# neoncloud/mdctGAN

Hardware: AMD Instinct MI355X
Metric: train steps/sec (G+D) VCTK 12k->48k (higher is better)
Workload: dtype f32; 1 GPU; configs[1]: netG=global ngf=64 n_blocks_global=9 n_blocks_attn_g=0 num_D=2, per-GPU batch 8 x 32512 samples (128 frames x 256 bins), 12k->48k, fp32; global_batch=8, segment_length=32512, parallelism=dp1, launch=hipGraph replay

## Files before the change

include/mdctgan_hip.h:

```cpp
#ifndef MDCTGAN_HIP_H
#define MDCTGAN_HIP_H

#include <stddef.h>

#ifdef __cplusplus
extern "C" {
#endif

#define MG_OK 0
#define MG_ERR_ARG (-1)
#define MG_ERR_UNSUPPORTED (-2)

#define MG_CODEC_RAW 0
#define MG_CODEC_ARCSINH 1
#define MG_CODEC_RANGE 2

#define MG_ACT_NONE 0
#define MG_ACT_RELU 1
#define MG_ACT_LRELU02 2
#define MG_ACT_TANH 3

int mg_abi_version(void);
int mg_conv_geom_size(void);

// ... 195 lines not shown
int mg_conv_fwd_instnorm_w(const mg_conv_geom* g, const float* x, const float* w, const float* bias, float* y_raw, float eps,
                           int act, const float* residual, float* y, float* mean, float* rstd, void* workspace,
                           size_t workspace_bytes, void* stream, const mg_wino_tiles* wt);
int mg_conv_wino_md_from_norm_ok(const mg_conv_geom* g);
int mg_instnorm_bwd_wino_md(const mg_conv_geom* g, const float* gy, const float* y_raw, const float* mean, const float* rstd,
                            int act, float* md, void* stream);
int mg_conv_fwd_instnorm_h(const mg_conv_geom* g, const float* x, const float* w, const float* bias, float* y_raw, float eps,
                           int act, const float* residual, float* y, float* mean, float* rstd, void* workspace,
                           size_t workspace_bytes, void* stream, const mg_wino_tiles* tiles, void* y16);
int mg_conv_wino_vnext_ok(const mg_conv_geom* g);
int mg_conv_fwd_instnorm_next(const mg_conv_geom* g, const float* x, const float* w, const float* bias, float* y_raw, float eps,
                              int act, const float* residual, float* y, float* mean, float* rstd, void* workspace,
                              size_t workspace_bytes, void* stream, const mg_wino_tiles* tiles, float* v_next, int next_reflect);
int mg_conv_dgrad_w(const mg_conv_geom* g, const float* dy, const float* w, const float* bias, float* dx, int act,
                    void* workspace, size_t workspace_bytes, void* stream, const mg_wino_tiles* tiles);
int mg_conv_wgrad(const mg_conv_geom* g, const float* x, const float* dy, float* dw, float* dbias, int accumulate,
                  void* workspace, size_t workspace_bytes, void* stream);
size_t mg_conv_wgrad_workspace(const mg_conv_geom* g);
int mg_conv_wgrad_w(const mg_conv_geom* g, const float* x, const float* dy, float* dw, float* dbias, int accumulate,
                    void* workspace, size_t workspace_bytes, void* stream, const mg_wino_tiles* tiles);
int mg_conv_wgrad_checks_finite(const mg_conv_geom* g);
int mg_conv_wgrad_chk(const mg_conv_geom* g, const float* x, const float* dy, float* dw, float* dbias, int accumulate,
                      void* workspace, size_t workspace_bytes, void* stream, const mg_wino_tiles* tiles, float* found_inf);
int mg_conv_wgrad_h16_ok(const mg_conv_geom* g);
int mg_conv_wgrad_h16(const mg_conv_geom* g, const float* x, const float* dy, void* dw16, int accumulate, void* workspace,
                      size_t workspace_bytes, void* stream, float* found_inf);
typedef struct {
    float* m;
    float* v;
    float* u;
// ... 128 lines not shown
```

mdctgan_amd/_lib.py:

```python
from __future__ import annotations

import ctypes as C
import os

import torch

_HERE = os.path.dirname(os.path.abspath(__file__))
LIB_PATH = os.environ.get("MDCTGAN_HIP_LIB", os.path.join(_HERE, "libmdctgan_hip.so"))

MG_CODEC_RAW, MG_CODEC_ARCSINH, MG_CODEC_RANGE, MG_CODEC_DB, MG_CODEC_EXPLICIT = 0, 1, 2, 3, 4
ACT_NONE, ACT_RELU, ACT_LRELU02, ACT_TANH = 0, 1, 2, 3


class HipLibraryError(RuntimeError):
    pass


class ConvGeom(C.Structure):
    _fields_ = [(n, C.c_int) for n in
                ("B", "H", "W", "Ci", "OH", "OW", "Co", "KH", "KW", "stride", "pad", "reflect", "precision")]


PRECISION_F32, PRECISION_F16 = 0, 1

# ... 7 lines not shown


_W = C.POINTER(WinoTiles)


class LossItem(C.Structure):
    _fields_ = [("a", C.c_void_p), ("b", C.c_void_p), ("grad", C.c_void_p), ("n", C.c_longlong), ("zero_tail", C.c_longlong)]


class WinoAdam(C.Structure):
    _fields_ = [("m", C.c_void_p), ("v", C.c_void_p), ("u", C.c_void_p), ("state", C.c_void_p),
                ("beta1", C.c_float), ("beta2", C.c_float), ("eps", C.c_float), ("grad_scale", C.c_float)]


_WA = C.POINTER(WinoAdam)


class ResampleBank(C.Structure):
    _fields_ = [("kern", C.c_void_p), ("orig", C.c_int), ("new_", C.c_int), ("width", C.c_int)]


_RB = C.POINTER(ResampleBank)

SIGNATURES = {
    "mg_abi_version": (_i, []),
    "mg_conv_geom_size": (_i, []),
    "mg_mdct4_forward": (_i, [_p, _i, _i, _i, _p, _p, _p, _i, _f, _f, _f, _f, _f, _i, _p, _p, _p, _p, _p, _p, _p, _p]),
    "mg_mdct4_num_frames": (_i, [_i, _i]),
    "mg_dct4_image": (_i, [_p, _p, _p]),
    "mg_dct4_image_floats": (_ll, [_i]),
# ... 13 lines not shown
    "mg_imdct4_pow2_stitched": (_i, [_p, _i, _i, _i, _p, _p, _i, _f, _f, _f, _f, _f, _p, _p, _p, _ll, _i, _i, _ll, _i, _i, _p]),
    "mg_conv_fwd": (_i, [_G, _p, _p, _p, _p, _i, _p, _sz, _p]),
    "mg_conv_fwd_workspace": (_sz, [_G]),
    "mg_conv_wino_weights_bytes": (_sz, [_G]),
    "mg_conv_wino_prepare": (_i, [_G, _p, _p, _p]),
    "mg_conv_wino_tiles_bytes": (_sz, [_G, _i]),
    "mg_conv_fwd_w": (_i, [_G, _p, _p, _p, _p, _i, _p, _sz, _p, _W]),
    "mg_conv_fwd_instnorm_workspace": (_sz, [_G]),
    "mg_conv_wino_md_from_norm_ok": (_i, [_G]),
    "mg_instnorm_bwd_wino_md": (_i, [_G, _p, _p, _p, _p, _i, _p, _p]),
    "mg_conv_fwd_instnorm_w": (_i, [_G, _p, _p, _p, _p, _f, _i, _p, _p, _p, _p, _p, _sz, _p, _W]),
    "mg_conv_fwd_instnorm_h": (_i, [_G, _p, _p, _p, _p, _f, _i, _p, _p, _p, _p, _p, _sz, _p, _W, _p]),
    "mg_conv_fwd_instnorm_next": (_i, [_G, _p, _p, _p, _p, _f, _i, _p, _p, _p, _p, _p, _sz, _p, _W, _p, _i]),
    "mg_conv_wino_vnext_ok": (_i, [_G]),
    "mg_conv_dgrad_w": (_i, [_G, _p, _p, _p, _p, _i, _p, _sz, _p, _W]),
    "mg_conv_wgrad_w": (_i, [_G, _p, _p, _p, _p, _i, _p, _sz, _p, _W]),
    "mg_conv_wgrad_chk": (_i, [_G, _p, _p, _p, _p, _i, _p, _sz, _p, _W, _p]),
    "mg_conv_wgrad_checks_finite": (_i, [_G]),
    "mg_conv_wgrad_adam_ok": (_i, [_G]),
    "mg_conv_wgrad_adam_w": (_i, [_G, _p, _p, _p, _WA, _p, _sz, _p, _W]),
    "mg_conv_dgrad": (_i, [_G, _p, _p, _p, _p, _i, _p, _sz, _p]),
    "mg_conv_dgrad_workspace": (_sz, [_G]),
    "mg_conv_wgrad": (_i, [_G, _p, _p, _p, _p, _i, _p, _sz, _p]),
    "mg_conv_wgrad_workspace": (_sz, [_G]),
    "mg_conv_plan_name": (_i, [_i, _G, C.c_char_p, _i]),
    "mg_conv_plan_splits": (_i, [_i, _G]),
    "mg_conv_plan_order": (_i, [_i, _G, C.POINTER(C.c_int), C.POINTER(C.c_int)]),
    "mg_conv_plan_flops": (C.c_double, [_i, _G]),
    "mg_probe_arm": (None, [_p, _p]),
    "mg_resample_length": (_ll, [_ll, _i, _i]),
# ... 192 lines not shown
```

mdctgan_amd/csrc/conv_igemm.hip:

```cpp
#include "common.h"
#include "mdctgan_hip.h"
#include "internal.h"
#include <stdio.h>
#include <stdlib.h>
#include <cstring>
#include <type_traits>
#include <map>
#include <mutex>
#include <tuple>
#include <hip/hip_ext.h>

namespace {

constexpr int BK = 16;

struct Geom {
    int B, H, W, Ci, OH, OW, Co, KH, KW, s, p, reflect;
};

struct Batch {
    long long sa, sw, so;
    int wino_perm;
};
__device__ __forceinline__ int wino_flip(int z) {
// ... 1573 lines not shown
    }
    const dim3 grid(wino_grid((size_t)w.T * g->Co / w.f.vec));
    if (w.r == R_WINO)
        hipLaunchKernelGGL(wino_output_xform_kernel, grid, dim3(256), 0, st, (const float*)Mx, g->B, w.TH, w.TW, g->Co, bias, act, y,
                           (int)w.hp);
    else if (w.r == R_WINO4)
        hipLaunchKernelGGL(wino4_output_xform_kernel, grid, dim3(256), 0, st, (const float*)Mx, g->B, w.TH, w.TW, g->Co, bias, act, y);
    else
        hipLaunchKernelGGL(wino42_output_xform_kernel, grid, dim3(256), 0, st, (const float*)Mx, g->B, g->OH, g->OW, w.TH, w.TW, g->Co,
                           bias, act, y);
    MG_CHECK_LAUNCH();
    return MG_OK;
}

int wino_dgrad(const WinoGeo& w, const mg_conv_geom* g, const float* dy, const float* wt, const float* bias, float* dx, int act,
               float* ws, hipStream_t st, const float* u_pre, float* md_keep, const float** addend) {
    const WinoGemm s = wino_gemm_plan(w, 1, g);
    const WinoWs o = wino_ws(w, s, 1, g);
    float* U = u_pre ? const_cast<float*>(u_pre) : ws + o.u;
    float* Md = md_keep ? md_keep : ws + o.md;
    float* dV = ws + o.dv;
    float* dd = ws + o.dd;
    if (!u_pre) wino_xform_u(w, g, wt, U, st);
    if (dy) wino_xform_md(w, g, dy, Md, st);
    wino_gemm(w, s, 1, g, Md, U, dV, ws + o.part, st);
    if (w.r == R_WINO && !w.hp && wino_dd_gather_ok(g->H, g->W, g->Ci)) {
        const int ts = w.TH * w.TW;
        const size_t lds = (size_t)ts * 16 * 8 * sizeof(float4);
        const dim3 grid(g->Ci / 32, g->B);
        const float* add = *addend;
        *addend = nullptr;
        auto go = [&](auto kern) {
            hipFuncSetAttribute((const void*)kern, hipFuncAttributeMaxDynamicSharedMemorySize, (int)lds);
            hipLaunchKernelGGL(kern, grid, dim3(256), lds, st, (const float*)dV, g->B, g->H, g->W, g->Ci, g->reflect, bias, act, dx, add);
        };
        if (ts <= 32) go(wino_dd_gather_kernel<1>); else go(wino_dd_gather_kernel<2>);
        MG_CHECK_LAUNCH();
        return MG_OK;
    }
    const dim3 grid(wino_grid((size_t)w.T * w.Kc / w.f.vec)), gx(wino_grid((size_t)g->B * g->H * g->W * g->Ci / 4));
    if (w.r == R_WINO) {
        hipLaunchKernelGGL(wino_dd_xform_kernel, grid, dim3(256), 0, st, (const float*)dV, w.T, w.Kc, dd);
        hipLaunchKernelGGL(wino_dx_gather_kernel, gx, dim3(256), 0, st, (const float*)dd, g->B, g->H, g->W, g->Ci, g->reflect, bias,
                           act, dx, (int)w.hp);
    } else {
        hipLaunchKernelGGL(wino4_dd_xform_kernel, grid, dim3(256), 0, st, (const float*)dV, w.T, w.Kc, dd);
        if (w.r == R_WINO4)
            hipLaunchKernelGGL(wino4_dx_gather_kernel, gx, dim3(256), 0, st, (const float*)dd, g->B, g->H, g->W, g->Ci, w.TH, w.TW, dx);
        else
            hipLaunchKernelGGL(wino42_dx_gather_kernel, gx, dim3(256), 0, st, (const float*)dd, g->B, g->H, g->W, g->Ci, w.TH, w.TW, dx);
    }
    MG_CHECK_LAUNCH();
    return MG_OK;
}
// ... 360 lines not shown
int mg_instnorm_bwd_wino_md(const mg_conv_geom* g, const float* gy, const float* y_raw, const float* mean, const float* rstd,
                            int act, float* md, void* stream) {
    if (!gy || !y_raw || !mean || !rstd || !md) return MG_ERR_ARG;
    if (!mg_conv_wino_md_from_norm_ok(g)) return MG_ERR_UNSUPPORTED;
    if (act != MG_ACT_NONE && act != MG_ACT_RELU && act != MG_ACT_LRELU02) return MG_ERR_UNSUPPORTED;
    if (!aligned16(gy) || !aligned16(y_raw) || !aligned16(mean) || !aligned16(rstd) || !aligned16(md)) return MG_ERR_ARG;
    const WinoGeo d = wino_geo(R_WINO, g);
    const dim3 grid(g->Co / 32, g->B);
    const int nt = (d.TH * d.TW + 31) / 32;
    hipStream_t st = (hipStream_t)stream;
#define MG_NORM_BWD_DY(NT_) hipLaunchKernelGGL(wino_norm_bwd_dy_kernel<NT_>, grid, dim3(256), 0, st, gy, y_raw, mean, rstd, g->B, d.TH, d.TW, g->Co, act, md)
    if (nt == 1) MG_NORM_BWD_DY(1); else if (nt == 2) MG_NORM_BWD_DY(2); else if (nt == 3) MG_NORM_BWD_DY(3); else if (nt == 4) MG_NORM_BWD_DY(4); else MG_NORM_BWD_DY(5);
#undef MG_NORM_BWD_DY
    MG_CHECK_LAUNCH();
    return MG_OK;
}
size_t mg_conv_fwd_instnorm_workspace(const mg_conv_geom* g) {
    if (!geom_ok(g)) return 0;
    const size_t a = mg_conv_fwd_workspace(g), b = mg_instnorm_workspace(g->B, g->OH * g->OW, g->Co);
    return a > b ? a : b;
}
int mg_conv_fwd_instnorm_w(const mg_conv_geom* g, const float* x, const float* w, const float* bias, float* y_raw, float eps,
                           int act, const float* residual, float* y, float* mean, float* rstd, void* workspace,
                           size_t workspace_bytes, void* stream, const mg_wino_tiles* wt) {
    return mg_conv_fwd_instnorm_h(g, x, w, bias, y_raw, eps, act, residual, y, mean, rstd, workspace, workspace_bytes, stream, wt, nullptr);
}
static bool wino_vnext_ok(const mg_conv_geom* g) {
    return wino_norm_ok(g) && wino_out_norm_next_ok(g->OH / 2, g->OW / 2, g->Co) && g->Co % 16 == 0;
}
int mg_conv_wino_vnext_ok(const mg_conv_geom* g) { return g && wino_vnext_ok(g) ? 1 : 0; }
// ... 436 lines not shown
```

mdctgan_amd/csrc/wino.h:

```cpp
#pragma once
#include "adam.h"

namespace {

__device__ __forceinline__ void bt4(const float4 d0, const float4 d1, const float4 d2, const float4 d3, float4 (&o)[4]) {
    o[0] = make_float4(d0.x - d2.x, d0.y - d2.y, d0.z - d2.z, d0.w - d2.w);
    o[1] = make_float4(d1.x + d2.x, d1.y + d2.y, d1.z + d2.z, d1.w + d2.w);
    o[2] = make_float4(d2.x - d1.x, d2.y - d1.y, d2.z - d1.z, d2.w - d1.w);
    o[3] = make_float4(d1.x - d3.x, d1.y - d3.y, d1.z - d3.z, d1.w - d3.w);
}
__device__ __forceinline__ float4 f4add(float4 a, float4 b) { return make_float4(a.x + b.x, a.y + b.y, a.z + b.z, a.w + b.w); }
__device__ __forceinline__ float4 f4sub(float4 a, float4 b) { return make_float4(a.x - b.x, a.y - b.y, a.z - b.z, a.w - b.w); }
__device__ __forceinline__ float4 f4scale(float4 a, float s) { return make_float4(a.x * s, a.y * s, a.z * s, a.w * s); }
__device__ __forceinline__ float4 f4neg(float4 a) { return make_float4(-a.x, -a.y, -a.z, -a.w); }

__global__ void wino_input_xform_kernel(const float* __restrict__ x, int B, int H, int W, int C, int TH, int TW,
                                        int org, int reflect, float* __restrict__ V) {
    const int C4 = C / 4;
    const size_t T = (size_t)B * TH * TW, total = T * C4;
    for (size_t i = (size_t)blockIdx.x * blockDim.x + threadIdx.x; i < total; i += (size_t)gridDim.x * blockDim.x) {
        const int c4 = (int)(i % C4);
        const size_t t = i / C4;
        const int tx = (int)(t % TW), ty = (int)((t / TW) % TH), b = (int)(t / ((size_t)TW * TH));
        float4 d[4][4];
// ... 246 lines not shown
                }
#pragma unroll
                for (int r = 0; r < 4; ++r) {
                    float4 o[4];
                    bt4(tmp[r][0], tmp[r][1], tmp[r][2], tmp[r][3], o);
#pragma unroll
                    for (int c = 0; c < 4; ++c)
                        *reinterpret_cast<float4*>(nrm.v_next + ((size_t)(r * 4 + c) * T + t) * C + c0) = o[c];
                }
            }
        }
    }
}
inline bool wino_out_norm_next_ok(int TH, int TW, int C) { return C % 32 == 0 && TH * TW <= 64; }

template <int NT>
__global__ __launch_bounds__(256) void wino_norm_bwd_dy_kernel(const float* __restrict__ gy, const float* __restrict__ x,
                                                               const float* __restrict__ mean, const float* __restrict__ rstd,
                                                               int B, int TH, int TW, int C, int act, float* __restrict__ Md) {
    __shared__ double red[2][32][32];
    const int cq = threadIdx.x & 7, tl = threadIdx.x >> 3;
    const int b = blockIdx.y, c0 = blockIdx.x * 32 + 4 * cq;
    const int Ts = TH * TW, HW = 4 * Ts;
    const size_t T = (size_t)B * Ts;
    const float4 mu4 = ld4(mean + (size_t)b * C + c0), rs4 = ld4(rstd + (size_t)b * C + c0);
    const float mu[4] = {mu4.x, mu4.y, mu4.z, mu4.w}, rs[4] = {rs4.x, rs4.y, rs4.z, rs4.w};
    float xh[NT][4][4], gq[NT][4][4];
    double s1[4] = {0, 0, 0, 0}, s2[4] = {0, 0, 0, 0};
#pragma unroll
    for (int i = 0; i < NT; ++i) {
        const int tile = tl + 32 * i;
        if (tile < Ts) {
            const int ty = tile / TW, tx = tile - ty * TW;
#pragma unroll
            for (int q = 0; q < 4; ++q) {
                const size_t off = ((size_t)(b * 2 * TH + 2 * ty + (q >> 1)) * (2 * TW) + 2 * tx + (q & 1)) * C + c0;
                float xv[4], gv[4];
                *reinterpret_cast<float4*>(xv) = ld4(x + off);
                *reinterpret_cast<float4*>(gv) = ld4(gy + off);
#pragma unroll
                for (int j = 0; j < 4; ++j) {
                    xh[i][q][j] = (xv[j] - mu[j]) * rs[j];
                    const float d = act == MG_ACT_RELU ? (xh[i][q][j] > 0.0f ? 1.0f : 0.0f)
                                  : act == MG_ACT_LRELU02 ? (xh[i][q][j] > 0.0f ? 1.0f : 0.2f) : 1.0f;
                    gq[i][q][j] = gv[j] * d;
                    s1[j] += (double)gq[i][q][j];
                    s2[j] += (double)gq[i][q][j] * (double)xh[i][q][j];
                }
            }
        } else {
#pragma unroll
            for (int q = 0; q < 4; ++q)
#pragma unroll
                for (int j = 0; j < 4; ++j) xh[i][q][j] = gq[i][q][j] = 0.f;
// ... 42 lines not shown
                for (int j = 0; j < 4; ++j) o[j] = rs[j] * (gq[i][q][j] - m1[j] - xh[i][q][j] * m2[j]);
                d[q] = make_float4(o[0], o[1], o[2], o[3]);
            }
            const float4 y00 = d[0], y01 = d[1], y10 = d[2], y11 = d[3];
            float4 tmp[4][2] = {{y00, y01}, {f4add(y00, y10), f4add(y01, y11)}, {f4sub(y00, y10), f4sub(y01, y11)},
                                {f4neg(y10), f4neg(y11)}};
            const size_t t = (size_t)b * Ts + tile;
#pragma unroll
            for (int r = 0; r < 4; ++r) {
                const float4 o[4] = {tmp[r][0], f4add(tmp[r][0], tmp[r][1]), f4sub(tmp[r][0], tmp[r][1]), f4neg(tmp[r][1])};
#pragma unroll
                for (int c = 0; c < 4; ++c) *reinterpret_cast<float4*>(Md + ((size_t)(r * 4 + c) * T + t) * C + c0) = o[c];
            }
        }
    }
}
inline bool wino_out_norm_ok(int TH, int TW, int C) {
    return C % 32 == 0 && TH * TW <= 160;
}

__global__ void wino_fold_reflect_kernel(const float* __restrict__ dxp, int B, int H, int W, int C,
                                         float* __restrict__ dx, int round_f16 = 0, const float* __restrict__ addend = nullptr) {
    const int C4 = C / 4;
    const size_t total = (size_t)B * H * W * C4;
    for (size_t i = (size_t)blockIdx.x * blockDim.x + threadIdx.x; i < total; i += (size_t)gridDim.x * blockDim.x) {
        const int c4 = (int)(i % C4);
        size_t r = i / C4;
        const int ix = (int)(r % W); r /= W;
        const int iy = (int)(r % H);
        const int b = (int)(r / H);
// ... 79 lines not shown
        const int ny = wino_sources(iy, H, TH, reflect, ty, ry), nx = wino_sources(ix, W, TW, reflect, tx, rx);
        float4 s = bias ? ld4(bias + 4 * c4) : zero4();
        float4 acc = zero4();
        for (int a = 0; a < ny; ++a)
            for (int c = 0; c < nx; ++c)
                add4(acc, ld4(dd + (((size_t)(b * TH + ty[a]) * TW + tx[c]) * 16 + ry[a] * 4 + rx[c]) * C + 4 * c4));
        add4(s, acc);
        s.x = apply_act(s.x, act); s.y = apply_act(s.y, act); s.z = apply_act(s.z, act); s.w = apply_act(s.w, act);
        if (round_f16) { s.x = round_h(s.x); s.y = round_h(s.y); s.z = round_h(s.z); s.w = round_h(s.w); }
        *reinterpret_cast<float4*>(dx + i * 4) = s;
    }
}


template <int NT>
__global__ __launch_bounds__(256) void wino_dd_gather_kernel(const float* __restrict__ dV, int B, int H, int W, int C, int reflect,
                                                             const float* __restrict__ bias, int act, float* __restrict__ dx,
                                                             const float* __restrict__ addend) {
    extern __shared__ __attribute__((aligned(16))) float4 wdg_lds[];
    const int cq = threadIdx.x & 7, tl = threadIdx.x >> 3;
    const int b = blockIdx.y, c0 = blockIdx.x * 32 + 4 * cq;
    const int TH = H / 2, TW = W / 2, Ts = TH * TW;
    const size_t T = (size_t)B * Ts;
#pragma unroll
    for (int i = 0; i < NT; ++i) {
        const int tile = tl + 32 * i;
        if (tile < Ts) {
            const size_t t = (size_t)b * Ts + tile;
            float4 v[4][4];
#pragma unroll
            for (int r = 0; r < 4; ++r)
#pragma unroll
                for (int c = 0; c < 4; ++c) v[r][c] = ld4(dV + ((size_t)(r * 4 + c) * T + t) * C + c0);
            float4 tmp[4][4];
#pragma unroll
            for (int c = 0; c < 4; ++c) {
                float4 o[4];
                b4(v[0][c], v[1][c], v[2][c], v[3][c], o);
                tmp[0][c] = o[0]; tmp[1][c] = o[1]; tmp[2][c] = o[2]; tmp[3][c] = o[3];
            }
#pragma unroll
            for (int r = 0; r < 4; ++r) {
                float4 o[4];
                b4(tmp[r][0], tmp[r][1], tmp[r][2], tmp[r][3], o);
#pragma unroll
                for (int c = 0; c < 4; ++c) wdg_lds[(tile * 16 + r * 4 + c) * 8 + cq] = o[c];
            }
        }
    }
    __syncthreads();
    const int HW = H * W;
    const float4 bv = bias ? ld4(bias + c0) : zero4();
    for (int p = tl; p < HW; p += 32) {
        const int iy = p / W, ix = p - iy * W;
        int ty[3], ry[3], tx[3], rx[3];
        const int ny = wino_sources(iy, H, TH, reflect, ty, ry), nx = wino_sources(ix, W, TW, reflect, tx, rx);
        float4 s = bv;
        float4 acc = zero4();
        for (int a = 0; a < ny; ++a)
            for (int c = 0; c < nx; ++c) add4(acc, wdg_lds[((ty[a] * TW + tx[c]) * 16 + ry[a] * 4 + rx[c]) * 8 + cq]);
        add4(s, acc);
        s.x = apply_act(s.x, act); s.y = apply_act(s.y, act); s.z = apply_act(s.z, act); s.w = apply_act(s.w, act);
        if (addend) add4(s, ld4(addend + ((size_t)b * HW + p) * C + c0));
        *reinterpret_cast<float4*>(dx + ((size_t)b * HW + p) * C + c0) = s;
    }
}
inline bool wino_dd_gather_ok(int H, int W, int C) {
    return C % 32 == 0 && (H / 2) * (W / 2) <= 64;
}

__global__ void wino_dy_xform_kernel(const float* __restrict__ dy, int B, int TH, int TW, int C, float* __restrict__ Md) {
    const int C4 = C / 4;
    const size_t T = (size_t)B * TH * TW, total = T * C4;
    for (size_t i = (size_t)blockIdx.x * blockDim.x + threadIdx.x; i < total; i += (size_t)gridDim.x * blockDim.x) {
        const int c4 = (int)(i % C4);
        const size_t t = i / C4;
        const int tx = (int)(t % TW), ty = (int)((t / TW) % TH), b = (int)(t / ((size_t)TW * TH));
        const float* p = dy + ((size_t)(b * 2 * TH + 2 * ty) * (2 * TW) + 2 * tx) * C + 4 * c4;
        const float4 y00 = ld4(p), y01 = ld4(p + C), y10 = ld4(p + (size_t)2 * TW * C), y11 = ld4(p + (size_t)2 * TW * C + C);
        float4 tmp[4][2] = {{y00, y01}, {f4add(y00, y10), f4add(y01, y11)}, {f4sub(y00, y10), f4sub(y01, y11)},
// ... 119 lines not shown
```

mdctgan_amd/functional.py:

```python
from __future__ import annotations

import os

import torch

from . import _lib, amp, ops
from ._lib import ACT_LRELU02, ACT_NONE, ACT_RELU, ACT_TANH

CL = torch.channels_last


def to_cl(x: torch.Tensor) -> torch.Tensor:
    if x.dtype != torch.float32:
        x = x.float()
    return x.contiguous(memory_format=CL)


def nhwc_view(x):
    return x.permute(0, 2, 3, 1)


def nchw_view(y):
    return y.permute(0, 3, 1, 2)

# ... 38 lines not shown

def _attach_wino_v(t, v, key):
    t._mg_wino_v = (v, t.data_ptr(), t._version, key)
    WINO_NEXT_STATS["made"] += 1
    return t


def _wino_v_of(t, key):
    rec = getattr(t, "_mg_wino_v", None)
    if rec is None:
        return None
    v, ptr, ver, k = rec
    if t.data_ptr() != ptr or t._version != ver or k != key or not t.is_contiguous(memory_format=CL):
        return None
    return v


def grad_buffer(p: torch.nn.Parameter):
    fresh = getattr(p, "_mg_fresh", True)
    if p.grad is None:
        p.grad = torch.empty_like(p)
        fresh = True
    p._mg_fresh = False
    p._mg_inf_checked = False
    return p.grad, (not fresh)


def grad_buffer16(p: torch.nn.Parameter):
    fresh = getattr(p, "_mg_fresh", True)
    p._mg_fresh = False
# ... 395 lines not shown
                ops.colsum(nhwc_view(gy).reshape(-1, g.Ci), bbuf, bacc)
        _notify(weight)
        if bias is not None and bias.requires_grad:
            _notify(bias)
    return dx


def conv2d(x, weight, bias, stride=1, padding=0, reflect=False, act=ACT_NONE, weight_grad=True):
    return _ConvFn.apply(x, weight, bias, (stride, padding, bool(reflect), act, False, weight_grad))


def conv_transpose2d(x, weight, bias, stride=2, padding=1, act=ACT_NONE, weight_grad=True):
    return _ConvFn.apply(x, weight, bias, (stride, padding, False, act, True, weight_grad))


class _ConvInstNormFn(torch.autograd.Function):

    @staticmethod
    def forward(ctx, x, weight, bias, residual, cfg):
        x = to_cl(x)
        pad, reflect, weight_grad, act, eps = cfg[:5]
        ctx.skip = cfg[5] if len(cfg) > 5 else None
        res = to_cl(residual) if residual is not None else None
        B, _, H, W = x.shape
        w = weight.detach()
        assert w.is_contiguous(memory_format=CL), "conv weights must be channels_last (OHWI) tensors"
        g = ops.conv_geom(B, H, W, w.shape[1], w.shape[0], w.shape[2], w.shape[3], 1, pad, reflect, amp.current_precision())
        _tag_g16(g, weight, bias, weight_grad)
        if ctx.needs_input_grad[0]:
            u = _weight_image(g, weight, weight_grad)
# ... 17 lines not shown
        v_next = None
        if next_reflect is not None and ops.wino_vnext_ok(g) and os.environ.get("MG_NO_WINO_NEXT", "0") != "1":
            v_next = torch.empty(16 * B * (g.OH // 2) * (g.OW // 2) * g.Co, dtype=torch.float32, device=x.device)
        y16 = (torch.empty(B * g.OH * g.OW * g.Co, dtype=torch.float16, device=x.device)
               if _want_h16(B, g.OH * g.OW, g.Co) else None)
        need_raw = bool(cfg[6]) and any(ctx.needs_input_grad) if len(cfg) > 6 else any(ctx.needs_input_grad)
        y, y_raw, mean, rstd = ops.conv_fwd_instnorm(g, nhwc_view(x), w, bias.detach() if bias is not None else None, act,
                                                     nhwc_view(res) if res is not None else None, eps, u, v, v_filled, y16,
                                                     need_raw=need_raw, v_next=v_next, next_reflect=bool(next_reflect))
        ctx.u, ctx.v = u, (v if (weight_grad and weight.requires_grad) else None)
        ctx.g, ctx.cfg = g, (1, pad, reflect, ACT_NONE, False, weight_grad)
        ctx.weight, ctx.bias, ctx.norm_act = weight, bias, act
        if need_raw:
            ctx.save_for_backward(x, nchw_view(y_raw), mean, rstd)
        out = _attach_h16(nchw_view(y), y16)
        if v_next is not None:
            _attach_wino_v(out, v_next, (B, g.OH, g.OW, g.Co, bool(next_reflect), g.precision))
        return out

    @staticmethod
    def backward(ctx, gy):
        x, y_raw, mean, rstd = ctx.saved_tensors
        gy = to_cl(gy)
        dres = gy if ctx.needs_input_grad[3] else None
        skip_g = None
        if ctx.skip is not None:
            role, holder = ctx.skip
            if role == "give" and dres is not None:
                holder.g, dres = dres, None
            elif role == "take":
                skip_g, holder.g = holder.g, None
        g, weight, bias = ctx.g, ctx.weight, ctx.bias
        weight_grad = ctx.cfg[5]
        dead_bias = bias is None or not bias.requires_grad or (getattr(bias, "_mg_zero_grad", False) and not COMPUTE_DEAD_BIAS_GRADS)
        u, v = getattr(ctx, "u", None), getattr(ctx, "v", None)
        if (ctx.needs_input_grad[0] and weight_grad is True and weight.requires_grad and dead_bias and u is not None
                and v is not None and ops.wino_md_from_norm_ok(g)):
            _, md = ops.wino_tile_buffers(g, gy.device, want_v=False)
            ops.instnorm_bwd_wino_md(g, nhwc_view(gy), nhwc_view(y_raw), mean, rstd, ctx.norm_act, md)
            w = weight.detach()
            dx = nchw_view(ops.conv_dgrad(g, None, w, u=u, md_out=md,
                                          add=nhwc_view(skip_g) if skip_g is not None else None))
            if bias is not None and bias.requires_grad:
                _zero_grad_bias(bias)
            if not _wgrad_fused(u, g, weight, None, None, v, md):
                wbuf, wacc = grad_buffer(weight)
                ops.conv_wgrad(g, None, None, wbuf, None, wacc, v=v, md=md)
            ctx.u = ctx.v = None
            _notify(weight)
            if bias is not None and bias.requires_grad:
                _notify(bias)
            return dx, None, None, dres, None
        d16 = (torch.empty(gy.numel(), dtype=torch.float16, device=gy.device)
               if (_want_h16(g.B, g.OH * g.OW, g.Co, g.precision == _lib.PRECISION_F16) and ops.precast_ok(1, g)) else None)
        d_raw = _attach_h16(nchw_view(ops.instnorm_bwd(nhwc_view(gy), nhwc_view(y_raw), mean, rstd, ctx.norm_act, dx16=d16)), d16)
        dx = _conv_backward(ctx, d_raw, x, None, add=nhwc_view(skip_g) if (skip_g is not None and ctx.needs_input_grad[0]) else None)
        if skip_g is not None and dx is None:
# ... 452 lines not shown
```

mdctgan_amd/ops.py:

```python
from __future__ import annotations

import torch

from . import _lib
from ._lib import ACT_LRELU02, ACT_NONE, ACT_RELU, ACT_TANH, ConvGeom


def conv_geom(B, H, W, Ci, Co, KH, KW, stride, pad, reflect, precision=0) -> ConvGeom:
    OH = (H + 2 * pad - KH) // stride + 1
    OW = (W + 2 * pad - KW) // stride + 1
    return ConvGeom(B, H, W, Ci, OH, OW, Co, KH, KW, stride, pad, int(bool(reflect)), int(precision))


def _ws(nbytes, dev):
    return _lib.workspace(nbytes, dev)


PROFILER = None


def plan_name(pass_id: int, g: ConvGeom) -> str:
    import ctypes
    buf = ctypes.create_string_buffer(96)
    _lib.check(_lib.load().mg_conv_plan_name(pass_id, g, buf, 96), "mg_conv_plan_name")
# ... 126 lines not shown

def instnorm_bwd_wino_md(g: ConvGeom, gy, y_raw, mean, rstd, act, md):
    _lib.check(_lib.load().mg_instnorm_bwd_wino_md(g, _lib.ptr(gy), _lib.ptr(y_raw), _lib.ptr(mean), _lib.ptr(rstd), act,
                                                   _lib.ptr(md), _lib.stream()), "mg_instnorm_bwd_wino_md")


def conv_dgrad(g: ConvGeom, dy, w, bias=None, act=ACT_NONE, u=None, md_out=None, out=None, add=None, md_filled=False):
    lib = _lib.load()
    dx = torch.empty(g.B, g.H, g.W, g.Ci, dtype=torch.float32, device=w.device) if out is None else out
    ws = _ws(lib.mg_conv_dgrad_workspace(g), w.device)
    if PROFILER is not None:
        PROFILER.begin(1, g)
    _lib.check(lib.mg_conv_dgrad_w(g, _lib.ptr(dy), _lib.ptr(w), _lib.ptr(bias), _lib.ptr(dx), act, _lib.ptr(ws),
                                   ws.numel(), _lib.stream(), _tiles(u, None, md_out, add, TILES_MD_FILLED if md_filled else 0)),
               "mg_conv_dgrad")
    if PROFILER is not None:
        PROFILER.end()
    return dx


def conv_wgrad(g: ConvGeom, x, dy, dw, dbias=None, accumulate=False, v=None, md=None, found_inf=None):
    lib = _lib.load()
    nbytes = lib.mg_conv_wgrad_workspace(g)
    ws = _ws(nbytes, dw.device)
    if PROFILER is not None:
        PROFILER.begin(2, g)
    _lib.check(lib.mg_conv_wgrad_chk(g, _lib.ptr(x), _lib.ptr(dy), _lib.ptr(dw), _lib.ptr(dbias), int(accumulate),
                                     _lib.ptr(ws), ws.numel(), _lib.stream(), _tiles(None, v, md), _lib.ptr(found_inf)),
               "mg_conv_wgrad")
    if PROFILER is not None:
# ... 398 lines not shown
```

Before: 91.02 steps/s.

## Fuse Winograd dgrad gather with producer's instance-norm backward into next md tiles

When a conv+instnorm layer feeds another Winograd conv+instnorm layer, the consumer's dgrad gather kernel now also runs the producer's instance-norm backward. It builds the producer's Winograd md tile image directly from the dx values it holds in LDS. The producer's backward pass then reuses that md image through a handover record and skips its separate instnorm_bwd_wino_md launch and the re-read of dx from global memory. In exchange the gather kernel uses more registers and LDS. It also relies on Python-side bookkeeping of pointers and versions that can fall back to the old path.

```diff
diff --git a/include/mdctgan_hip.h b/include/mdctgan_hip.h
--- a/include/mdctgan_hip.h
+++ b/include/mdctgan_hip.h
@@ -233,6 +233,16 @@
                               size_t workspace_bytes, void* stream, const mg_wino_tiles* tiles, float* v_next, int next_reflect);
 int mg_conv_dgrad_w(const mg_conv_geom* g, const float* dy, const float* w, const float* bias, float* dx, int act,
                     void* workspace, size_t workspace_bytes, void* stream, const mg_wino_tiles* tiles);
+typedef struct {
+    const float* y_raw;
+    const float* mean;
+    const float* rstd;
+    int act;
+    float* md_out;
+} mg_wino_bwd_next;
+int mg_conv_dgrad_wino_next_ok(const mg_conv_geom* g, const mg_conv_geom* g_prod);
+int mg_conv_dgrad_wino_next(const mg_conv_geom* g, const float* w, float* dx, void* workspace, size_t workspace_bytes, void* stream,
+                            const mg_wino_tiles* tiles, const mg_conv_geom* g_prod, const mg_wino_bwd_next* next);
 int mg_conv_wgrad(const mg_conv_geom* g, const float* x, const float* dy, float* dw, float* dbias, int accumulate,
                   void* workspace, size_t workspace_bytes, void* stream);
 size_t mg_conv_wgrad_workspace(const mg_conv_geom* g);
diff --git a/mdctgan_amd/_lib.py b/mdctgan_amd/_lib.py
--- a/mdctgan_amd/_lib.py
+++ b/mdctgan_amd/_lib.py
@@ -45,6 +45,13 @@
 
 
 _WA = C.POINTER(WinoAdam)
+
+
+class WinoBwdNext(C.Structure):
+    _fields_ = [("y_raw", C.c_void_p), ("mean", C.c_void_p), ("rstd", C.c_void_p), ("act", C.c_int), ("md_out", C.c_void_p)]
+
+
+_WN = C.POINTER(WinoBwdNext)
 
 
 class ResampleBank(C.Structure):
@@ -88,6 +95,8 @@
     "mg_conv_fwd_instnorm_next": (_i, [_G, _p, _p, _p, _p, _f, _i, _p, _p, _p, _p, _p, _sz, _p, _W, _p, _i]),
     "mg_conv_wino_vnext_ok": (_i, [_G]),
     "mg_conv_dgrad_w": (_i, [_G, _p, _p, _p, _p, _i, _p, _sz, _p, _W]),
+    "mg_conv_dgrad_wino_next_ok": (_i, [_G, _G]),
+    "mg_conv_dgrad_wino_next": (_i, [_G, _p, _p, _p, _sz, _p, _W, _G, _WN]),
     "mg_conv_wgrad_w": (_i, [_G, _p, _p, _p, _p, _i, _p, _sz, _p, _W]),
     "mg_conv_wgrad_chk": (_i, [_G, _p, _p, _p, _p, _i, _p, _sz, _p, _W, _p]),
     "mg_conv_wgrad_checks_finite": (_i, [_G]),
diff --git a/mdctgan_amd/csrc/conv_igemm.hip b/mdctgan_amd/csrc/conv_igemm.hip
--- a/mdctgan_amd/csrc/conv_igemm.hip
+++ b/mdctgan_amd/csrc/conv_igemm.hip
@@ -1611,7 +1611,8 @@
 }
 
 int wino_dgrad(const WinoGeo& w, const mg_conv_geom* g, const float* dy, const float* wt, const float* bias, float* dx, int act,
-               float* ws, hipStream_t st, const float* u_pre, float* md_keep, const float** addend) {
+               float* ws, hipStream_t st, const float* u_pre, float* md_keep, const float** addend,
+               const mg_wino_bwd_next* nx = nullptr) {
     const WinoGemm s = wino_gemm_plan(w, 1, g);
     const WinoWs o = wino_ws(w, s, 1, g);
     float* U = u_pre ? const_cast<float*>(u_pre) : ws + o.u;
@@ -1631,10 +1632,17 @@
             hipFuncSetAttribute((const void*)kern, hipFuncAttributeMaxDynamicSharedMemorySize, (int)lds);
             hipLaunchKernelGGL(kern, grid, dim3(256), lds, st, (const float*)dV, g->B, g->H, g->W, g->Ci, g->reflect, bias, act, dx, add);
         };
-        if (ts <= 32) go(wino_dd_gather_kernel<1>); else go(wino_dd_gather_kernel<2>);
+        auto go_next = [&](auto kern) {
+            hipFuncSetAttribute((const void*)kern, hipFuncAttributeMaxDynamicSharedMemorySize, (int)lds);
+            hipLaunchKernelGGL(kern, grid, dim3(256), lds, st, (const float*)dV, g->B, g->H, g->W, g->Ci, g->reflect, dx, add, nx->y_raw,
+                               nx->mean, nx->rstd, nx->act, nx->md_out);
+        };
+        if (nx) { if (ts <= 32) go_next(wino_dd_gather_norm_dy_kernel<1>); else go_next(wino_dd_gather_norm_dy_kernel<2>); }
+        else if (ts <= 32) go(wino_dd_gather_kernel<1>); else go(wino_dd_gather_kernel<2>);
         MG_CHECK_LAUNCH();
         return MG_OK;
     }
+    if (nx) return MG_ERR_UNSUPPORTED;
     const dim3 grid(wino_grid((size_t)w.T * w.Kc / w.f.vec)), gx(wino_grid((size_t)g->B * g->H * g->W * g->Ci / 4));
     if (w.r == R_WINO) {
         hipLaunchKernelGGL(wino_dd_xform_kernel, grid, dim3(256), 0, st, (const float*)dV, w.T, w.Kc, dd);
@@ -2025,6 +2033,25 @@
 #undef MG_NORM_BWD_DY
     MG_CHECK_LAUNCH();
     return MG_OK;
+}
+int mg_conv_dgrad_wino_next_ok(const mg_conv_geom* g, const mg_conv_geom* gp) {
+    if (!g || !gp || !wino_norm_ok(g) || !wino_norm_ok(gp)) return 0;
+    if (conv_route(1, g) != R_WINO || !wino_dd_gather_ok(g->H, g->W, g->Ci)) return 0;
+    return gp->Co == g->Ci && gp->B == g->B && gp->OH == g->H && gp->OW == g->W ? 1 : 0;
+}
+int mg_conv_dgrad_wino_next(const mg_conv_geom* g, const float* w, float* dx, void* workspace, size_t workspace_bytes, void* stream,
+                            const mg_wino_tiles* wt, const mg_conv_geom* gp, const mg_wino_bwd_next* nx) {
+    if (!g || !gp || !nx) return MG_ERR_ARG;
+    if (!mg_conv_dgrad_wino_next_ok(g, gp)) return MG_ERR_UNSUPPORTED;
+    if (nx->act != MG_ACT_NONE && nx->act != MG_ACT_RELU && nx->act != MG_ACT_LRELU02) return MG_ERR_UNSUPPORTED;
+    if (!w || !dx || !wt || !wt->md || !nx->y_raw || !nx->mean || !nx->rstd || !nx->md_out) return MG_ERR_ARG;
+    if (!wino_tiles_ok(g, wt) || (wt->add && !aligned16(wt->add))) return MG_ERR_ARG;
+    if (!aligned16(w) || !aligned16(dx) || !aligned16(nx->y_raw) || !aligned16(nx->mean) || !aligned16(nx->rstd) || !aligned16(nx->md_out))
+        return MG_ERR_ARG;
+    if (!workspace || !aligned16(workspace) || workspace_bytes < mg_conv_dgrad_workspace(g)) return MG_ERR_ARG;
+    const float* add = wt->add;
+    return wino_dgrad(wino_geo(R_WINO, g), g, nullptr, w, nullptr, dx, MG_ACT_NONE, (float*)workspace, (hipStream_t)stream, wt->u, wt->md,
+                      &add, nx);
 }
 size_t mg_conv_fwd_instnorm_workspace(const mg_conv_geom* g) {
     if (!geom_ok(g)) return 0;
diff --git a/mdctgan_amd/csrc/wino.h b/mdctgan_amd/csrc/wino.h
--- a/mdctgan_amd/csrc/wino.h
+++ b/mdctgan_amd/csrc/wino.h
@@ -284,11 +284,10 @@
 }
 inline bool wino_out_norm_next_ok(int TH, int TW, int C) { return C % 32 == 0 && TH * TW <= 64; }
 
-template <int NT>
-__global__ __launch_bounds__(256) void wino_norm_bwd_dy_kernel(const float* __restrict__ gy, const float* __restrict__ x,
-                                                               const float* __restrict__ mean, const float* __restrict__ rstd,
-                                                               int B, int TH, int TW, int C, int act, float* __restrict__ Md) {
-    __shared__ double red[2][32][32];
+template <int NT, class LoadX, class LoadGy>
+__device__ __forceinline__ void wino_norm_bwd_dy_slab(LoadX load_x, LoadGy load_gy, const float* __restrict__ mean,
+                                                      const float* __restrict__ rstd, int B, int TH, int TW, int C, int act,
+                                                      float* __restrict__ Md, double (&red)[2][32][32]) {
     const int cq = threadIdx.x & 7, tl = threadIdx.x >> 3;
     const int b = blockIdx.y, c0 = blockIdx.x * 32 + 4 * cq;
     const int Ts = TH * TW, HW = 4 * Ts;
@@ -306,8 +305,8 @@
             for (int q = 0; q < 4; ++q) {
                 const size_t off = ((size_t)(b * 2 * TH + 2 * ty + (q >> 1)) * (2 * TW) + 2 * tx + (q & 1)) * C + c0;
                 float xv[4], gv[4];
-                *reinterpret_cast<float4*>(xv) = ld4(x + off);
-                *reinterpret_cast<float4*>(gv) = ld4(gy + off);
+                *reinterpret_cast<float4*>(xv) = load_x(i, q, off);
+                *reinterpret_cast<float4*>(gv) = load_gy(i, q, off);
 #pragma unroll
                 for (int j = 0; j < 4; ++j) {
                     xh[i][q][j] = (xv[j] - mu[j]) * rs[j];
@@ -380,6 +379,14 @@
             }
         }
     }
+}
+template <int NT>
+__global__ __launch_bounds__(256) void wino_norm_bwd_dy_kernel(const float* __restrict__ gy, const float* __restrict__ x,
+                                                               const float* __restrict__ mean, const float* __restrict__ rstd,
+                                                               int B, int TH, int TW, int C, int act, float* __restrict__ Md) {
+    __shared__ double red[2][32][32];
+    wino_norm_bwd_dy_slab<NT>([&](int, int, size_t off) { return ld4(x + off); }, [&](int, int, size_t off) { return ld4(gy + off); },
+                              mean, rstd, B, TH, TW, C, act, Md, red);
 }
 inline bool wino_out_norm_ok(int TH, int TW, int C) {
     return C % 32 == 0 && TH * TW <= 160;
@@ -489,6 +496,50 @@
 
 
 template <int NT>
+__device__ __forceinline__ void wino_dd_patches(const float* __restrict__ dV, int b, int Ts, size_t T, int C, float4* lds) {
+    const int cq = threadIdx.x & 7, tl = threadIdx.x >> 3;
+    const int c0 = blockIdx.x * 32 + 4 * cq;
+#pragma unroll
+    for (int i = 0; i < NT; ++i) {
+        const int tile = tl + 32 * i;
+        if (tile < Ts) {
+            const size_t t = (size_t)b * Ts + tile;
+            float4 v[4][4];
+#pragma unroll
+            for (int r = 0; r < 4; ++r)
+#pragma unroll
+                for (int c = 0; c < 4; ++c) v[r][c] = ld4(dV + ((size_t)(r * 4 + c) * T + t) * C + c0);
+            float4 tmp[4][4];
+#pragma unroll
+            for (int c = 0; c < 4; ++c) {
+                float4 o[4];
+                b4(v[0][c], v[1][c], v[2][c], v[3][c], o);
+                tmp[0][c] = o[0]; tmp[1][c] = o[1]; tmp[2][c] = o[2]; tmp[3][c] = o[3];
+            }
+#pragma unroll
+            for (int r = 0; r < 4; ++r) {
+                float4 o[4];
+                b4(tmp[r][0], tmp[r][1], tmp[r][2], tmp[r][3], o);
+#pragma unroll
+                for (int c = 0; c < 4; ++c) lds[(tile * 16 + r * 4 + c) * 8 + cq] = o[c];
+            }
+        }
+    }
+}
+__device__ __forceinline__ float4 wino_dd_pixel(const float4* lds, int p, int H, int W, int TH, int TW, int reflect, float4 bv, int act) {
+    const int cq = threadIdx.x & 7;
+    const int iy = p / W, ix = p - iy * W;
+    int ty[3], ry[3], tx[3], rx[3];
+    const int ny = wino_sources(iy, H, TH, reflect, ty, ry), nx = wino_sources(ix, W, TW, reflect, tx, rx);
+    float4 s = bv;
+    float4 acc = zero4();
+    for (int a = 0; a < ny; ++a)
+        for (int c = 0; c < nx; ++c) add4(acc, lds[((ty[a] * TW + tx[c]) * 16 + ry[a] * 4 + rx[c]) * 8 + cq]);
+    add4(s, acc);
+    s.x = apply_act(s.x, act); s.y = apply_act(s.y, act); s.z = apply_act(s.z, act); s.w = apply_act(s.w, act);
+    return s;
+}
+template <int NT>
 __global__ __launch_bounds__(256) void wino_dd_gather_kernel(const float* __restrict__ dV, int B, int H, int W, int C, int reflect,
                                                              const float* __restrict__ bias, int act, float* __restrict__ dx,
                                                              const float* __restrict__ addend) {
@@ -496,49 +547,61 @@
     const int cq = threadIdx.x & 7, tl = threadIdx.x >> 3;
     const int b = blockIdx.y, c0 = blockIdx.x * 32 + 4 * cq;
     const int TH = H / 2, TW = W / 2, Ts = TH * TW;
-    const size_t T = (size_t)B * Ts;
-#pragma unroll
-    for (int i = 0; i < NT; ++i) {
-        const int tile = tl + 32 * i;
-        if (tile < Ts) {
-            const size_t t = (size_t)b * Ts + tile;
-            float4 v[4][4];
-#pragma unroll
-            for (int r = 0; r < 4; ++r)
-#pragma unroll
-                for (int c = 0; c < 4; ++c) v[r][c] = ld4(dV + ((size_t)(r * 4 + c) * T + t) * C + c0);
-            float4 tmp[4][4];
-#pragma unroll
-            for (int c = 0; c < 4; ++c) {
-                float4 o[4];
-                b4(v[0][c], v[1][c], v[2][c], v[3][c], o);
-                tmp[0][c] = o[0]; tmp[1][c] = o[1]; tmp[2][c] = o[2]; tmp[3][c] = o[3];
-            }
-#pragma unroll
-            for (int r = 0; r < 4; ++r) {
-                float4 o[4];
-                b4(tmp[r][0], tmp[r][1], tmp[r][2], tmp[r][3], o);
-#pragma unroll
-                for (int c = 0; c < 4; ++c) wdg_lds[(tile * 16 + r * 4 + c) * 8 + cq] = o[c];
-            }
-        }
-    }
+    wino_dd_patches<NT>(dV, b, Ts, (size_t)B * Ts, C, wdg_lds);
     __syncthreads();
     const int HW = H * W;
     const float4 bv = bias ? ld4(bias + c0) : zero4();
     for (int p = tl; p < HW; p += 32) {
-        const int iy = p / W, ix = p - iy * W;
-        int ty[3], ry[3], tx[3], rx[3];
-        const int ny = wino_sources(iy, H, TH, reflect, ty, ry), nx = wino_sources(ix, W, TW, reflect, tx, rx);
-        float4 s = bv;
-        float4 acc = zero4();
-        for (int a = 0; a < ny; ++a)
-            for (int c = 0; c < nx; ++c) add4(acc, wdg_lds[((ty[a] * TW + tx[c]) * 16 + ry[a] * 4 + rx[c]) * 8 + cq]);
-        add4(s, acc);
-        s.x = apply_act(s.x, act); s.y = apply_act(s.y, act); s.z = apply_act(s.z, act); s.w = apply_act(s.w, act);
+        float4 s = wino_dd_pixel(wdg_lds, p, H, W, TH, TW, reflect, bv, act);
         if (addend) add4(s, ld4(addend + ((size_t)b * HW + p) * C + c0));
         *reinterpret_cast<float4*>(dx + ((size_t)b * HW + p) * C + c0) = s;
     }
+}
+template <int NT>
+__global__ __launch_bounds__(256) void wino_dd_gather_norm_dy_kernel(const float* __restrict__ dV, int B, int H, int W, int C, int reflect,
+                                                                     float* __restrict__ dx, const float* __restrict__ addend,
+                                                                     const float* __restrict__ x, const float* __restrict__ mean,
+                                                                     const float* __restrict__ rstd, int act, float* __restrict__ Md) {
+    extern __shared__ __attribute__((aligned(16))) float4 wdg_lds[];
+    __shared__ double red[2][32][32];
+    const int cq = threadIdx.x & 7, tl = threadIdx.x >> 3;
+    const int b = blockIdx.y, c0 = blockIdx.x * 32 + 4 * cq;
+    const int TH = H / 2, TW = W / 2, Ts = TH * TW, HW = H * W;
+    float4 xr[NT][4];
+#pragma unroll
+    for (int i = 0; i < NT; ++i) {
+        const int tile = tl + 32 * i;
+        const int ty = tile / TW, tx = tile - ty * TW;
+#pragma unroll
+        for (int q = 0; q < 4; ++q)
+            xr[i][q] = tile < Ts ? ld4(x + ((size_t)(b * H + 2 * ty + (q >> 1)) * W + 2 * tx + (q & 1)) * C + c0) : zero4();
+    }
+    wino_dd_patches<NT>(dV, b, Ts, (size_t)B * Ts, C, wdg_lds);
+    __syncthreads();
+    float4 px[4 * NT];
+#pragma unroll
+    for (int k = 0; k < 4 * NT; ++k) {
+        const int p = tl + 32 * k;
+        if (p < HW) {
+            float4 s = wino_dd_pixel(wdg_lds, p, H, W, TH, TW, reflect, zero4(), MG_ACT_NONE);
+            if (addend) add4(s, ld4(addend + ((size_t)b * HW + p) * C + c0));
+            *reinterpret_cast<float4*>(dx + ((size_t)b * HW + p) * C + c0) = s;
+            px[k] = s;
+        }
+    }
+    __syncthreads();
+#pragma unroll
+    for (int k = 0; k < 4 * NT; ++k) {
+        const int p = tl + 32 * k;
+        if (p < HW) wdg_lds[p * 8 + cq] = px[k];
+    }
+    __syncthreads();
+    wino_norm_bwd_dy_slab<NT>([&](int i, int q, size_t) { return xr[i][q]; },
+                              [&](int i, int q, size_t) {
+                                  const int tile = tl + 32 * i, ty = tile / TW, tx = tile - ty * TW;
+                                  return wdg_lds[((2 * ty + (q >> 1)) * W + 2 * tx + (q & 1)) * 8 + cq];
+                              },
+                              mean, rstd, B, TH, TW, C, act, Md, red);
 }
 inline bool wino_dd_gather_ok(int H, int W, int C) {
     return C % 32 == 0 && (H / 2) * (W / 2) <= 64;
diff --git a/mdctgan_amd/functional.py b/mdctgan_amd/functional.py
--- a/mdctgan_amd/functional.py
+++ b/mdctgan_amd/functional.py
@@ -76,6 +76,47 @@
     if t.data_ptr() != ptr or t._version != ver or k != key or not t.is_contiguous(memory_format=CL):
         return None
     return v
+
+
+WINO_BWD_NEXT_STATS = {"made": 0, "used": 0}
+
+
+class _BwdHandover:
+    __slots__ = ("g", "y_raw", "mean", "rstd", "act", "md", "dx", "dx_version")
+
+    def __init__(self, g, y_raw, mean, rstd, act):
+        self.g, self.y_raw, self.mean, self.rstd, self.act = g, y_raw, mean, rstd, act
+        self.md = self.dx = self.dx_version = None
+
+    def image_for(self, gy):
+        md, dx, ver = self.md, self.dx, self.dx_version
+        self.md = self.dx = self.dx_version = None
+        if (md is None or dx is None or gy.data_ptr() != dx.data_ptr() or gy._version != ver or gy.shape != dx.shape
+                or gy.stride() != dx.stride()):
+            return None
+        WINO_BWD_NEXT_STATS["used"] += 1
+        return md
+
+
+def _dgrad_handover(g, w, u, md, add, prev, out=None, md_prev=None):
+    if (prev is not None and os.environ.get("MG_NO_WINO_BWD_NEXT", "0") != "1"
+            and ops.wino_bwd_next_ok(g, prev.g)):
+        prev.md = md_prev if md_prev is not None else ops.wino_tile_buffers(prev.g, w.device, want_v=False)[1]
+        prev.dx = ops.conv_dgrad_next(g, w, u, md, prev.g, prev.y_raw, prev.mean, prev.rstd, prev.act, prev.md, add=add, out=out)
+        prev.dx_version = prev.dx._version
+        WINO_BWD_NEXT_STATS["made"] += 1
+        return prev.dx
+    return ops.conv_dgrad(g, None, w, u=u, md_out=md, add=add, out=out)
+
+
+def _bwd_handover_of(t):
+    rec = getattr(t, "_mg_wino_bwd", None)
+    if rec is None:
+        return None
+    h, ptr, ver = rec
+    if t.data_ptr() != ptr or t._version != ver or not t.is_contiguous(memory_format=CL):
+        return None
+    return h
 
 
 def grad_buffer(p: torch.nn.Parameter):
@@ -501,6 +542,10 @@
     return _ConvFn.apply(x, weight, bias, (stride, padding, False, act, True, weight_grad))
 
 
+def _dead_bias(bias):
+    return bias is None or not bias.requires_grad or (getattr(bias, "_mg_zero_grad", False) and not COMPUTE_DEAD_BIAS_GRADS)
+
+
 class _ConvInstNormFn(torch.autograd.Function):
 
     @staticmethod
@@ -548,8 +593,14 @@
         if need_raw:
             ctx.save_for_backward(x, nchw_view(y_raw), mean, rstd)
         out = _attach_h16(nchw_view(y), y16)
+        ctx.prev = _bwd_handover_of(x) if ctx.needs_input_grad[0] else None
+        ctx.handover = None
         if v_next is not None:
             _attach_wino_v(out, v_next, (B, g.OH, g.OW, g.Co, bool(next_reflect), g.precision))
+            if (need_raw and ctx.needs_input_grad[0] and weight_grad is True and weight.requires_grad and _dead_bias(bias)
+                    and u is not None and ctx.v is not None and ops.wino_md_from_norm_ok(g)):
+                ctx.handover = _BwdHandover(g, y_raw, mean, rstd, act)
+                out._mg_wino_bwd = (ctx.handover, out.data_ptr(), out._version)
         return out
 
     @staticmethod
@@ -566,15 +617,19 @@
                 skip_g, holder.g = holder.g, None
         g, weight, bias = ctx.g, ctx.weight, ctx.bias
         weight_grad = ctx.cfg[5]
-        dead_bias = bias is None or not bias.requires_grad or (getattr(bias, "_mg_zero_grad", False) and not COMPUTE_DEAD_BIAS_GRADS)
+        dead_bias = _dead_bias(bias)
         u, v = getattr(ctx, "u", None), getattr(ctx, "v", None)
+        mine, prev = ctx.handover, ctx.prev
+        ctx.handover = ctx.prev = None
         if (ctx.needs_input_grad[0] and weight_grad is True and weight.requires_grad and dead_bias and u is not None
                 and v is not None and ops.wino_md_from_norm_ok(g)):
-            _, md = ops.wino_tile_buffers(g, gy.device, want_v=False)
-            ops.instnorm_bwd_wino_md(g, nhwc_view(gy), nhwc_view(y_raw), mean, rstd, ctx.norm_act, md)
+            md = mine.image_for(nhwc_view(gy)) if mine is not None else None
+            if md is None:
+                _, md = ops.wino_tile_buffers(g, gy.device, want_v=False)
+                ops.instnorm_bwd_wino_md(g, nhwc_view(gy), nhwc_view(y_raw), mean, rstd, ctx.norm_act, md)
             w = weight.detach()
-            dx = nchw_view(ops.conv_dgrad(g, None, w, u=u, md_out=md,
-                                          add=nhwc_view(skip_g) if skip_g is not None else None))
+            add = nhwc_view(skip_g) if skip_g is not None else None
+            dx = nchw_view(_dgrad_handover(g, w, u, md, add, prev))
             if bias is not None and bias.requires_grad:
                 _zero_grad_bias(bias)
             if not _wgrad_fused(u, g, weight, None, None, v, md):
diff --git a/mdctgan_amd/ops.py b/mdctgan_amd/ops.py
--- a/mdctgan_amd/ops.py
+++ b/mdctgan_amd/ops.py
@@ -164,6 +164,28 @@
     _lib.check(lib.mg_conv_dgrad_w(g, _lib.ptr(dy), _lib.ptr(w), _lib.ptr(bias), _lib.ptr(dx), act, _lib.ptr(ws),
                                    ws.numel(), _lib.stream(), _tiles(u, None, md_out, add, TILES_MD_FILLED if md_filled else 0)),
                "mg_conv_dgrad")
+    if PROFILER is not None:
+        PROFILER.end()
+    return dx
+
+
+def wino_bwd_next_ok(g: ConvGeom, g_prod: ConvGeom) -> bool:
+    key = ("bn",) + tuple((q.B, q.H, q.W, q.Ci, q.Co, q.KH, q.KW, q.stride, q.pad, q.reflect, q.precision) for q in (g, g_prod))
+    hit = _CASTS.get(key)
+    if hit is None:
+        hit = _CASTS[key] = bool(_lib.load().mg_conv_dgrad_wino_next_ok(g, g_prod))
+    return hit
+
+
+def conv_dgrad_next(g: ConvGeom, w, u, md, g_prod: ConvGeom, y_raw, mean, rstd, act, md_prod, add=None, out=None):
+    lib = _lib.load()
+    dx = torch.empty(g.B, g.H, g.W, g.Ci, dtype=torch.float32, device=w.device) if out is None else out
+    ws = _ws(lib.mg_conv_dgrad_workspace(g), w.device)
+    nxt = _lib.WinoBwdNext(_lib.ptr(y_raw), _lib.ptr(mean), _lib.ptr(rstd), act, _lib.ptr(md_prod))
+    if PROFILER is not None:
+        PROFILER.begin(1, g)
+    _lib.check(lib.mg_conv_dgrad_wino_next(g, _lib.ptr(w), _lib.ptr(dx), _lib.ptr(ws), ws.numel(), _lib.stream(),
+                                           _tiles(u, None, md, add), g_prod, nxt), "mg_conv_dgrad_wino_next")
     if PROFILER is not None:
         PROFILER.end()
     return dx
```

Result: no change. 91.54 steps/s, median of 6 (+0.6%).
